# simonsysu/tfs

Hardware: AMD Instinct MI355X
Metric: GiB/s CRC32 verify, device-resident 64 KiB files; 1/2/4/8 MI355X (higher is better)
Workload: dtype u8

## Files before the change

### tfs_amd/csrc/tfs_ec_abi.cpp

```cpp
#include <hip/hip_runtime.h>

#include <cstdlib>
#include <cstring>
#include <mutex>
#include <vector>

#include "../../include/tfs_ec.h"
#include "crc_math.h"
#include "ec_math.h"

#include "ec_locate_plan.h"
#include "ec_marshal_plan.h"
#include "ec_read_plan.h"
#include "tfs_ec_device.h"

extern "C" int tfs_crc32_dev_malloc(tfs_crc_ctx* ctx, uint64_t bytes, void** d_ptr);
extern "C" int tfs_crc32_dev_free(tfs_crc_ctx* ctx, void* d_ptr);
extern "C" void* tfs_crc32_stream(tfs_crc_ctx* ctx);

using namespace tfsec;

namespace {
struct Plan {
  std::vector<int> sources, outputs;
// ... 147 lines not shown
    if (!dm[i]) dm[i] = ec->staging[p.sources[0]];
  rc = run_plan(ec, p, dm.data(), size, st);
  if (rc) return rc;
  for (int o : p.outputs)
    if (hipMemcpyAsync(members[o], dm[o], size_t(size), hipMemcpyDeviceToHost, st) != hipSuccess)
      return TFS_CRC_EXIT_DEVICE_ERROR;
  return hipStreamSynchronize(st) == hipSuccess ? TFS_SUCCESS : TFS_CRC_EXIT_DEVICE_ERROR;
}


const ReadTables& read_tables() {
  static const ReadTables* t = [] {
    ReadTables* r = new ReadTables();
    tfscrc::make_slice_tables(r->slice, 4);
    tfscrc::make_shift_table(r->step_packet, kReadStepPacket);
    tfscrc::make_shift_table(r->step_tile, kReadStepTile);
    const uint32_t g = tfscrc::x2nmodp(8, 0), gi = tfscrc::x2nmodp(0xFFFFFFFFull - 8, 0);
    r->xpow[kReadPowBias] = 1u << 31;
    for (int i = kReadPowBias + 1; i < kReadPowN; ++i) r->xpow[i] = tfscrc::multmodp(g, r->xpow[i - 1]);
    for (int i = kReadPowBias - 1; i >= 0; --i) r->xpow[i] = tfscrc::multmodp(gi, r->xpow[i + 1]);
    return r;
  }();
  return *t;
}

int upload_read_tables(tfs_ec* ec) {
  void* d = nullptr;
  const int rc = tfs_crc32_dev_malloc(ec->ctx, sizeof(ReadTables), &d);
  if (rc) return rc;
  if (hipMemcpy(d, &read_tables(), sizeof(ReadTables), hipMemcpyHostToDevice) != hipSuccess) {
    tfs_crc32_dev_free(ec->ctx, d);
    return TFS_CRC_EXIT_DEVICE_ERROR;
  }
  ec->d_read_tab = static_cast<ReadTables*>(d);
  return TFS_SUCCESS;
}

int check_read(tfs_ec* ec, void* const* members, const int* sizes, int size, int target, int* row) {
  const Plan& p = ec->dec;
  if (!p.valid || !ec->d_read_tab) return TFS_EXIT_MATRIX_INVALID;
  if (size < 0 || size % kUnit != 0) return TFS_EXIT_SIZE_INVALID;
  if (target < 0 || target >= ec->dn) return TFS_EXIT_PARAMETER_ERROR;
  *row = -1;
  for (size_t o = 0; o < p.outputs.size(); ++o)
    if (p.outputs[o] == target) *row = int(o);
  if (*row < 0) return TFS_EXIT_PARAMETER_ERROR;
  if (!members) return TFS_EXIT_DATA_INVALID;
  for (int s : p.sources)
    if (!members[s] || (sizes && sizes[s] < size)) return TFS_EXIT_DATA_INVALID;
  return TFS_SUCCESS;
}

int launch_read(tfs_ec* ec, void* const* members, int size, int row, const void* d_jobs, uint32_t n, void* d_out,
                uint64_t out_cap, uint32_t* d_out_crc, int32_t* d_out_status, uint32_t* d_n_bad, hipStream_t st) {
  const Plan& p = ec->dec;
  const int S = int(p.sources.size());
  ReadArgs a;
  memset(&a, 0, sizeof a);
  for (int s = 0; s < S; ++s) a.src[s] = static_cast<const uint8_t*>(members[p.sources[s]]);
  a.masks = p.d_masks + size_t(row) * 8 * size_t(S) * 8;
  a.tab = ec->d_read_tab;
  a.jobs = static_cast<const ReadJob*>(d_jobs);
  a.out = static_cast<uint8_t*>(d_out);
  a.out_cap = out_cap;
  a.out_crc = d_out_crc;
  a.out_status = d_out_status;
  a.n_bad = d_n_bad;
  a.n = n;
  a.S = uint32_t(S);
  a.size = size;
  return launch_ec_read(a, st) == hipSuccess ? TFS_SUCCESS : TFS_CRC_EXIT_DEVICE_ERROR;
}


const MarshalTables& marshal_tables() {
  static const MarshalTables* t = [] {
    MarshalTables* r = new MarshalTables();
    tfscrc::make_slice_tables(r->slice, 4);
    tfscrc::make_shift_table(r->step_packet, kReadStepPacket);
    const uint32_t g = tfscrc::x2nmodp(8, 0), gi = tfscrc::x2nmodp(0xFFFFFFFFull - 8, 0);
    r->xpow[kMarshalPowBias] = 1u << 31;
    for (int i = kMarshalPowBias + 1; i < kMarshalPowN; ++i) r->xpow[i] = tfscrc::multmodp(g, r->xpow[i - 1]);
    for (int i = kMarshalPowBias - 1; i >= 0; --i) r->xpow[i] = tfscrc::multmodp(gi, r->xpow[i + 1]);
    return r;
  }();
  return *t;
}

int chunk_check(tfs_ec_marshal* m, int offset, int len, hipStream_t want, hipStream_t* st) {
  if (!m || !m->ec) return TFS_EXIT_PARAMETER_ERROR;
  if (want == hipStreamPerThread) return TFS_EXIT_PARAMETER_ERROR;
  *st = want ? want : static_cast<hipStream_t>(tfs_crc32_stream(m->ec->ctx));
  if (m->stream_set && *st != m->stream) return TFS_EXIT_PARAMETER_ERROR;
  if (offset != m->next || len <= 0 || offset % 4096 != 0 || len % kUnit != 0 || len > m->total - offset)
    return TFS_EXIT_PARAMETER_ERROR;
  if (len % 4096 != 0 && offset + len != m->total) return TFS_EXIT_PARAMETER_ERROR;
  return TFS_SUCCESS;
}

int marshal_check(tfs_ec_marshal* m, void* const* members, int offset, int len, hipStream_t want, hipStream_t* st) {
  const int rc = chunk_check(m, offset, len, want, st);
  if (rc) return rc;
  if (!members) return TFS_EXIT_DATA_INVALID;
  for (int i = 0; i < m->ec->dn + m->ec->pn; ++i)
    if (!members[i]) return TFS_EXIT_DATA_INVALID;
  return TFS_SUCCESS;
}

int marshal_launch(tfs_ec_marshal* m, void* const* members, int offset, int len, hipStream_t st) {
  tfs_ec* ec = m->ec;
  const Plan& p = ec->enc;
  if (m->plan.recs.empty()) return run_plan(ec, p, members, len, st);
  const int S = int(p.sources.size());
  for (size_t o0 = 0; o0 < p.outputs.size(); o0 += kMaxOutGroup) {
    const int og = int(std::min<size_t>(kMaxOutGroup, p.outputs.size() - o0));
    MarshalArgs a;
    memset(&a, 0, sizeof a);
    for (int s = 0; s < S; ++s) a.ec.src[s] = static_cast<const uint8_t*>(members[p.sources[s]]);
    for (int o = 0; o < og; ++o) a.ec.dst[o] = static_cast<uint8_t*>(members[p.outputs[o0 + o]]);
    a.ec.masks = p.d_masks + o0 * 8 * size_t(S) * 8;
    a.ec.S = uint32_t(S);
    a.ec.units = uint64_t(len) / kUnit;
    if (o0) {
      if (launch_ec_apply(a.ec, og, 0, st) != hipSuccess) return TFS_CRC_EXIT_DEVICE_ERROR;
      continue;
    }
    a.tab = ec->d_marshal_tab;
    a.recs = m->d_recs;
    a.first = m->d_first;
    a.cont = m->d_cont;
    a.tail = m->d_tail;
    a.hdr = m->d_hdr;
    for (int s = 0; s < S; ++s) a.mend[s] = m->plan.mbegin[s + 1];
    a.tile0 = uint32_t(offset) >> 12;
    a.ntiles = m->plan.ntiles;
    if (launch_ec_marshal(a, og, st) != hipSuccess) return TFS_CRC_EXIT_DEVICE_ERROR;
  }
  return TFS_SUCCESS;
}


int reinstate_check(tfs_ec_reinstate* r, void* const* members, int offset, int len, hipStream_t want, hipStream_t* st) {
  if (!r) return TFS_EXIT_PARAMETER_ERROR;
  const int rc = chunk_check(&r->s, offset, len, want, st);
  if (rc) return rc;
  if (!members) return TFS_EXIT_DATA_INVALID;
  const Plan& p = r->s.ec->dec;
  for (int i : p.sources)
    if (!members[i]) return TFS_EXIT_DATA_INVALID;
  for (int i : p.outputs)
    if (!members[i]) return TFS_EXIT_DATA_INVALID;
  return TFS_SUCCESS;
}

int reinstate_launch(tfs_ec_reinstate* r, void* const* members, int offset, int len, hipStream_t st) {
  tfs_ec_marshal* m = &r->s;
  tfs_ec* ec = m->ec;
  const Plan& p = ec->dec;
  if (m->plan.recs.empty()) return run_plan(ec, p, members, len, st);
  const int S = int(p.sources.size()), dn = ec->dn;
  for (size_t o0 = 0; o0 < p.outputs.size(); o0 += kMaxOutGroup) {
    const int og = int(std::min<size_t>(kMaxOutGroup, p.outputs.size() - o0));
    ReinstateArgs a;
    memset(&a, 0, sizeof a);
    EcArgs& e = a.m.ec;
    for (int s = 0; s < S; ++s) e.src[s] = static_cast<const uint8_t*>(members[p.sources[s]]);
// ... 857 lines not shown
```

### tfs_amd/csrc/tfs_ec_device.h

```cpp
#pragma once
#include <hip/hip_runtime.h>
#include <stdint.h>

#include "ec_update_plan.h"

namespace tfsec {

constexpr int kMaxMembersDev = 12;
constexpr int kMaxOutGroup = 4;

struct EcArgs {
  const uint8_t* src[kMaxMembersDev];
  uint8_t* dst[kMaxOutGroup];
  const uint32_t* masks;
  uint32_t S;
  uint64_t units;
};

hipError_t launch_ec_apply(const EcArgs& a, int og, int variant, hipStream_t stream);

struct ReadJob {
  uint64_t file_id;
  uint64_t out_offset;
  int32_t offset, size;
  uint32_t flags, reserved;
};
static_assert(sizeof(ReadJob) == 32, "read job layout");
constexpr uint32_t kReadRange = 1u;
constexpr int kReadWaves = 8;
constexpr unsigned kReadMaxGrid = 4096;
constexpr uint32_t kReadStepPacket = 128, kReadStepTile = 4096u * kReadWaves - 896u;
constexpr int kReadPowBias = 4095;
constexpr int kReadPowN = kReadPowBias + 4096 * (kReadWaves - 1) + 3192 + 1;
struct ReadTables {
  uint32_t slice[4][256];
  uint32_t step_packet[4][256];
  uint32_t step_tile[4][256];
  uint32_t xpow[kReadPowN];
};
#ifdef __HIP__
__attribute__((host)) __attribute__((device))
#endif
inline int32_t read_job_check(const ReadJob& jb, int32_t member_size, uint64_t out_cap, uint32_t* A, uint32_t* E) {
  const int64_t cover_end = (int64_t(jb.offset) + int64_t(jb.size) + 1023) & ~int64_t(1023);
  if (jb.offset < 0 || jb.size < 0 || cover_end > int64_t(member_size)) return -1016;
  *A = uint32_t(jb.offset) & ~1023u;
  *E = uint32_t(cover_end);
  if ((jb.out_offset & 1023u) != 0u || jb.out_offset > out_cap || uint64_t(*E - *A) > out_cap - jb.out_offset)
    return -1016;
  if (!(jb.flags & kReadRange) && jb.size <= 36) return -8034;
  return 0;
}

struct ReadArgs {
  const uint8_t* src[kMaxMembersDev];
  const uint32_t* masks;
  const ReadTables* tab;
  const ReadJob* jobs;
  uint8_t* out;
  uint64_t out_cap;
  uint32_t* out_crc;
  int32_t* out_status;
  uint32_t* n_bad;
  uint32_t n, S;
  int32_t size;
};

hipError_t launch_ec_read(const ReadArgs& a, hipStream_t stream);

struct MarshalRec {
  uint32_t H, P1;
  uint32_t id_lo, id_hi;
};
constexpr int kMarshalPowBias = 4095;
constexpr int kMarshalPowN = kMarshalPowBias + 4096 + 1;
constexpr uint32_t kMarshalHdrWords = 9;
struct MarshalTables {
  uint32_t slice[4][256];
  uint32_t step_packet[4][256];
  uint32_t xpow[kMarshalPowN];
};
struct MarshalArgs {
  EcArgs ec;
  const MarshalTables* tab;
  const MarshalRec* recs;
  const uint32_t* first;
  uint32_t* cont;
  uint32_t* tail;
  uint32_t* hdr;
  uint32_t mend[kMaxMembersDev];
  uint32_t tile0;
  uint32_t ntiles;
};
hipError_t launch_ec_marshal(const MarshalArgs& a, int og, hipStream_t stream);

struct MarshalFoldArgs {
  const MarshalTables* tab;
  const MarshalRec* recs;
  const uint32_t* rec_member;
  const uint32_t* cont;
  const uint32_t* tail;
  const uint32_t* hdr;
  const uint32_t* pow_tile;
  uint32_t* out_crc;
  int32_t* out_status;
  uint32_t n, ntiles;
};
hipError_t launch_ec_marshal_fold(const MarshalFoldArgs& a, hipStream_t stream);

constexpr uint32_t kReinstateNoSlot = 0xFFFFFFFFu;
struct ReinstateArgs {
  MarshalArgs m;
  uint32_t src_slot[kMaxMembersDev];
  uint32_t out_slot[kMaxOutGroup];
};
hipError_t launch_ec_reinstate(const ReinstateArgs& a, int og, hipStream_t stream);

struct ScrubArgs {
  MarshalArgs m;
  const uint8_t* par[kMaxOutGroup];
  uint32_t* pbad;
  uint32_t o0;
};
hipError_t launch_ec_scrub(const ScrubArgs& a, int og, bool walk, hipStream_t stream);

struct ScrubCountArgs {
  const uint32_t* pbad;
  uint32_t* units;
  uint8_t* map;
  uint32_t ntiles;
};
hipError_t launch_ec_scrub_count(const ScrubCountArgs& a, int pn, hipStream_t stream);

struct LocateResult {
  int8_t kind, member;
  uint16_t parity, diff_bytes;
  uint8_t flags, zero;
};
static_assert(sizeof(LocateResult) == 8, "locate result layout");
constexpr int kLocateClean = 0, kLocateParity = 1, kLocateData = 2, kLocateNone = 3;
constexpr uint32_t kLocateConfirmed = 1u;
struct LocateArgs {
  const uint8_t* mem[kMaxMembersDev];
  const uint32_t* masks;
  const uint32_t* ratio;
  const uint32_t* inv0;
  const uint32_t* units;
  LocateResult* result;
  uint8_t* fixed;
  uint32_t n, dn, pn;
};
hipError_t launch_ec_locate(const LocateArgs& a, hipStream_t stream);

struct UpdateArgs {
  uint8_t* par[kMaxMembersDev];
  const uint32_t* masks;
  const uint32_t* units;
  const uint8_t* a;
  const uint8_t* b;
  uint32_t inl[kUpdateInline];
  uint32_t n, n_inline, dn, pn, member;
};
hipError_t launch_ec_update(const UpdateArgs& a, hipStream_t stream);

// ... 2 lines not shown
```

### tfs_amd/csrc/tfs_ec_kernels.hip

```cpp
#include <hip/hip_runtime.h>
#include <stdint.h>

#include "tfs_crc_device.h"
#include "tfs_ec_device.h"

namespace tfsec {

typedef unsigned int u32x2 __attribute__((ext_vector_type(2)));
typedef const __attribute__((address_space(1))) u32x2* gu64p;
typedef __attribute__((address_space(1))) u32x2* gu64wp;

__device__ __forceinline__ u32x2 ld64nt(const uint8_t* p) {
  return __builtin_nontemporal_load(reinterpret_cast<gu64p>(reinterpret_cast<uintptr_t>(p)));
}
__device__ __forceinline__ void st64nt(uint8_t* p, u32x2 v) {
  __builtin_nontemporal_store(v, reinterpret_cast<gu64wp>(reinterpret_cast<uintptr_t>(p)));
}
__device__ __forceinline__ uint32_t xand(uint32_t acc, uint32_t in, uint32_t m) {
  return __builtin_amdgcn_bitop3_b32(acc, in, m, 0x78);
}

template <int OG>
__device__ __forceinline__ void ec_apply_body(const EcArgs& a, const uint32_t* __restrict__ masks) {
  const int lane = threadIdx.x & 63;
// ... 314 lines not shown
            acc[r].x = xand(acc[r].x, in[c].x, mk);
            acc[r].y = xand(acc[r].y, in[c].y, mk);
          }
        }
#pragma unroll
        for (int c = 0; c < 8; ++c) in[c] = nx[c];
      }
      if (ok) {
#pragma unroll
        for (int r = 0; r < 8; ++r) st64nt(outp + (base - A) + 128u * r, acc[r]);
      }
      if (range) continue;
      if (t == 0) {
#pragma unroll
        for (int c = 0; c < 8; ++c) {
          const uint32_t q = base + 128u * c;
          if (q + 8u > H && q < P0) {
            const uint64_t v = uint64_t(acc[c].x) | (uint64_t(acc[c].y) << 32);
#pragma unroll
            for (int b = 0; b < 8; ++b) {
              const uint32_t p = q + uint32_t(b) - H;
              if (p < uint32_t(tfscrc::kFileInfoSize)) hdr8[p] = uint8_t(v >> (8 * b));
            }
          }
        }
      }
#pragma unroll
      for (int c = 0; c < 8; ++c) {
        const uint32_t q = base + 128u * c;
        uint32_t lo = acc[c].x, hi = acc[c].y;
        const int64_t sk = int64_t(P0) - int64_t(q), ek = int64_t(P1) - int64_t(q);
        if (sk > 0 || ek < 8) {
          const uint64_t mk = ek <= sk ? 0ull : rd_low_bytes(ek) & ~rd_low_bytes(sk);
          lo &= uint32_t(mk);
          hi &= uint32_t(mk >> 32);
        }
        const uint32_t piece = rd_slice4(sl, rd_slice4(sl, lo) ^ hi);
        crc = rd_lut4(c == 0 ? stt : stp, crc) ^ piece;
      }
    }
    if (range) {
      if (threadIdx.x == 0) {
        a.out_crc[j] = 0u;
        a.out_status[j] = tfscrc::kSuccess;
      }
      continue;
    }
    {
      const uint32_t tl = nt - 1u - ((nt - 1u - wv) & (kReadWaves - 1u));
      const int32_t dl = wv < nt ? int32_t(4096u * (nt - 1u - tl)) + 3192 - int32_t(1024u * u + off) : 0;
      const int32_t pad = int32_t(A + 4096u * nt - P1);
      crc = rd_multmodp(a.tab->xpow[kReadPowBias + dl - pad], crc);
#pragma unroll
      for (int m = 32; m >= 1; m >>= 1) crc ^= __shfl_xor(crc, m, 64);
      if (lane == 0) part[wv] = crc;
    }
    __syncthreads();
    if (threadIdx.x == 0) {
      uint32_t v = 0;
#pragma unroll
      for (int w = 0; w < kReadWaves; ++w) v ^= part[w];
      const uint64_t id = uint64_t(hdr[0]) | (uint64_t(hdr[1]) << 32);
      const int32_t fsize = int32_t(hdr[3]);
      const uint32_t fcrc = hdr[8];
      if (id != jb.file_id) status = tfscrc::kExitFileInfoError;
      else if (fsize != jb.size) status = tfscrc::kExitSyncFileError;
      else if (fcrc != v) status = tfscrc::kExitCheckCrcError;
      a.out_crc[j] = v;
      a.out_status[j] = status;
      if (status != tfscrc::kSuccess) ++bad;
    }
    __syncthreads();
  }
  if (threadIdx.x == 0 && bad && a.n_bad) atomicAdd(a.n_bad, bad);
}

hipError_t launch_ec_read(const ReadArgs& a, hipStream_t stream) {
  if (a.n == 0) return hipSuccess;
  const uint32_t blocks = a.n < kReadMaxGrid ? a.n : kReadMaxGrid;
  hipLaunchKernelGGL(ec_read_kernel, dim3(blocks), dim3(64 * kReadWaves), 0, stream, a);
  return hipGetLastError();
}

template <int OG>
__global__ void __launch_bounds__(256, OG <= 3 ? 4 : 3)
    ec_marshal_kernel(MarshalArgs a, const uint32_t* __restrict__ masks, const MarshalTables* __restrict__ tab,
                      const MarshalRec* __restrict__ recs, const uint32_t* __restrict__ first) {
  __shared__ uint32_t lt[2 * 1024];
  const uint32_t* sl = lt;
  const uint32_t* stp = lt + 1024;
  const int lane = threadIdx.x & 63;
  const uint32_t u = uint32_t(lane) >> 4;
  const uint32_t off = 8u * uint32_t(lane & 15);
  const uint32_t S = a.ec.S;
  const uint64_t ntl = (a.ec.units + 3) / 4;
  const uint64_t t = uint64_t(blockIdx.x) * 4u + __builtin_amdgcn_readfirstlane(threadIdx.x >> 6);
  const uint64_t unit = t * 4 + u;
  const bool ok = t < ntl && unit < a.ec.units;
  const uint64_t base = unit * 1024u + off;
  u32x2 in[8];
#pragma unroll
  for (int c = 0; c < 8; ++c) in[c] = ok ? ld64nt(a.ec.src[0] + base + 128u * c) : u32x2{0u, 0u};
  {
    const uint32_t* g = reinterpret_cast<const uint32_t*>(tab);
    for (uint32_t i = threadIdx.x; i < 2u * 1024u; i += 256u) lt[i] = g[i];
  }
  __syncthreads();
  if (t >= ntl) return;
  const uint32_t T = a.tile0 + uint32_t(t);
  const uint32_t tile_lo = T << 12, tile_hi = tile_lo + 4096u;
  const uint32_t q0 = tile_lo + 1024u * u + off;
  const int32_t dl = 3192 - int32_t(1024u * u + off);
  uint8_t* const hdr8 = reinterpret_cast<uint8_t*>(a.hdr);
  u32x2 acc[OG][8];
#pragma unroll
  for (int o = 0; o < OG; ++o)
#pragma unroll
    for (int r = 0; r < 8; ++r) acc[o][r] = u32x2{0u, 0u};
  for (uint32_t s = 0; s < S; ++s) {
    u32x2 nx[8];
    const bool more = s + 1 < S;
    const uint8_t* np = a.ec.src[more ? s + 1 : s];
#pragma unroll
    for (int c = 0; c < 8; ++c) nx[c] = (ok && more) ? ld64nt(np + base + 128u * c) : u32x2{0u, 0u};
#pragma unroll
    for (int o = 0; o < OG; ++o)
#pragma unroll
      for (int r = 0; r < 8; ++r) {
        const uint32_t* m = masks + ((uint32_t(o) * 8u + uint32_t(r)) * S + s) * 8u;
#pragma unroll
        for (int c = 0; c < 8; ++c) {
          const uint32_t mk = m[c];
          acc[o][r].x = xand(acc[o][r].x, in[c].x, mk);
          acc[o][r].y = xand(acc[o][r].y, in[c].y, mk);
        }
      }
    const uint32_t rend = a.mend[s];
    for (uint32_t r = __builtin_amdgcn_readfirstlane(first[size_t(s) * a.ntiles + T]); r < rend; ++r) {
      const uint32_t H = __builtin_amdgcn_readfirstlane(recs[r].H);
      const uint32_t P1 = __builtin_amdgcn_readfirstlane(recs[r].P1);
      if (H >= tile_hi) break;
      const uint32_t P0 = H + uint32_t(tfscrc::kFileInfoSize);
      const uint32_t live = 0u - uint32_t(P1 > tile_lo);
      if (P0 > tile_lo) {
#pragma unroll
        for (int c = 0; c < 8; ++c) {
          const uint32_t q = q0 + 128u * c;
          if (q + 8u > H && q < P0) {
            const uint64_t v = uint64_t(in[c].x & live) | (uint64_t(in[c].y & live) << 32);
#pragma unroll
            for (int b = 0; b < 8; ++b) {
              const uint32_t p = q + uint32_t(b) - H;
              if (p < uint32_t(tfscrc::kFileInfoSize)) hdr8[size_t(r) * (4u * kMarshalHdrWords) + p] = uint8_t(v >> (8 * b));
            }
          }
        }
      }
      if (P0 >= tile_hi) continue;
      uint32_t crc = 0;
      if (P0 <= tile_lo && P1 >= tile_hi) {
#pragma unroll
        for (int c = 0; c < 8; ++c) {
          const uint32_t piece = rd_slice4(sl, rd_slice4(sl, in[c].x & live) ^ (in[c].y & live));
          crc = c == 0 ? piece : rd_lut4(stp, crc) ^ piece;
        }
      } else {
#pragma unroll
        for (int c = 0; c < 8; ++c) {
          const uint32_t q = q0 + 128u * c;
          uint32_t lo = in[c].x & live, hi = in[c].y & live;
          const int64_t sk = int64_t(P0) - int64_t(q), ek = int64_t(P1) - int64_t(q);
          if (sk > 0 || ek < 8) {
            const uint64_t mk = ek <= sk ? 0ull : rd_low_bytes(ek) & ~rd_low_bytes(sk);
            lo &= uint32_t(mk);
            hi &= uint32_t(mk >> 32);
          }
          const uint32_t piece = rd_slice4(sl, rd_slice4(sl, lo) ^ hi);
          crc = c == 0 ? piece : rd_lut4(stp, crc) ^ piece;
        }
      }
      const bool on = P1 > tile_hi;
      const int32_t pad = P1 >= tile_hi ? 0 : int32_t(tile_hi - P1);
      crc = rd_multmodp(tab->xpow[kMarshalPowBias + dl - pad], crc);
#pragma unroll
      for (int m = 32; m >= 1; m >>= 1) crc ^= __shfl_xor(crc, m, 64);
      if (lane == 0) {
        if (on) a.cont[size_t(s) * a.ntiles + T] = crc;
        else a.tail[r] = crc;
      }
    }
#pragma unroll
    for (int c = 0; c < 8; ++c) in[c] = nx[c];
  }
  if (ok) {
#pragma unroll
    for (int o = 0; o < OG; ++o)
#pragma unroll
      for (int r = 0; r < 8; ++r) st64nt(a.ec.dst[o] + base + 128u * r, acc[o][r]);
  }
}

hipError_t launch_ec_marshal(const MarshalArgs& a, int og, hipStream_t stream) {
  if (a.ec.units == 0) return hipSuccess;
  const uint64_t ntl = (a.ec.units + 3) / 4;
  const dim3 g(static_cast<unsigned>((ntl + 3) / 4)), b(256);
  switch (og) {
    case 1: hipLaunchKernelGGL(ec_marshal_kernel<1>, g, b, 0, stream, a, a.ec.masks, a.tab, a.recs, a.first); break;
    case 2: hipLaunchKernelGGL(ec_marshal_kernel<2>, g, b, 0, stream, a, a.ec.masks, a.tab, a.recs, a.first); break;
    case 3: hipLaunchKernelGGL(ec_marshal_kernel<3>, g, b, 0, stream, a, a.ec.masks, a.tab, a.recs, a.first); break;
    default: hipLaunchKernelGGL(ec_marshal_kernel<4>, g, b, 0, stream, a, a.ec.masks, a.tab, a.recs, a.first); break;
  }
  return hipGetLastError();
}

__global__ void __launch_bounds__(256) ec_marshal_fold_kernel(MarshalFoldArgs a) {
  const uint32_t lane = threadIdx.x & 63u;
  const uint32_t r = blockIdx.x * 4u + __builtin_amdgcn_readfirstlane(threadIdx.x >> 6);
  if (r >= a.n) return;
  const MarshalRec rc = a.recs[r];
  const uint32_t P0 = rc.H + uint32_t(tfscrc::kFileInfoSize), P1 = rc.P1;
  const uint32_t t0 = P0 >> 12, tl = (P1 - 1u) >> 12;
  const uint32_t nc = tl - t0;
  uint32_t c = 0;
  if (nc) {
    const uint32_t* cont = a.cont + size_t(a.rec_member[r]) * a.ntiles;
    const uint32_t R = (nc + 63u) / 64u;
    const uint32_t b = min(t0 + lane * R, tl), e = min(b + R, tl);
    const uint32_t x4k = a.pow_tile[1];
    for (uint32_t t = b; t < e; ++t) c = rd_multmodp(x4k, c) ^ cont[t];
    c = rd_multmodp(a.pow_tile[tl - e], c);
#pragma unroll
    for (int m = 32; m >= 1; m >>= 1) c ^= __shfl_xor(c, m, 64);
  }
  if (lane == 0) {
    const uint32_t v = rd_multmodp(a.tab->xpow[kMarshalPowBias + int32_t(P1 - (tl << 12))], c) ^ a.tail[r];
    const uint32_t* h = a.hdr + size_t(r) * kMarshalHdrWords;
    const int32_t size = int32_t(P1 - rc.H);
    int32_t status = tfscrc::kSuccess;
    if (h[0] != rc.id_lo || h[1] != rc.id_hi) status = tfscrc::kExitFileInfoError;
    else if (int32_t(h[3]) != size) status = tfscrc::kExitSyncFileError;
    else if (h[8] != v) status = tfscrc::kExitCheckCrcError;
    a.out_crc[r] = v;
    a.out_status[r] = status;
  }
}

hipError_t launch_ec_marshal_fold(const MarshalFoldArgs& a, hipStream_t stream) {
  if (a.n == 0) return hipSuccess;
  hipLaunchKernelGGL(ec_marshal_fold_kernel, dim3((a.n + 3u) / 4u), dim3(256), 0, stream, a);
  return hipGetLastError();
}

struct ReinstateWalk {
  const uint32_t* sl;
  const uint32_t* stp;
  uint32_t T, tile_lo, tile_hi, q0, ntiles;
  int32_t dl;
  int lane;
};

template <bool QREC = false>
__device__ __forceinline__ void reinstate_walk(const u32x2 (&pc)[8], const ReinstateWalk& w, uint32_t slot, uint32_t rend,
                                               const MarshalTables* __restrict__ tab, const MarshalRec* __restrict__ recs,
                                               const uint32_t* __restrict__ first, uint32_t* cont, uint32_t* tail,
                                               uint8_t* hdr8) {
  const uint32_t tile_lo = w.tile_lo, tile_hi = w.tile_hi;
  for (uint32_t r = __builtin_amdgcn_readfirstlane(first[size_t(slot) * w.ntiles + w.T]); r < rend; ++r) {
    const uint32_t H = __builtin_amdgcn_readfirstlane(recs[r].H);
    const uint32_t P1 = __builtin_amdgcn_readfirstlane(recs[r].P1);
    if (H >= tile_hi) break;
    const uint32_t P0 = H + uint32_t(tfscrc::kFileInfoSize);
    const uint32_t live = 0u - uint32_t(P1 > tile_lo);
    const uint32_t q0 = QREC ? w.q0 + ~live : w.q0;
    if (P0 > tile_lo) {
#pragma unroll
      for (int c = 0; c < 8; ++c) {
        const uint32_t q = q0 + 128u * c;
        if (q + 8u > H && q < P0) {
          const uint64_t v = uint64_t(pc[c].x & live) | (uint64_t(pc[c].y & live) << 32);
#pragma unroll
          for (int b = 0; b < 8; ++b) {
            const uint32_t p = q + uint32_t(b) - H;
            if (p < uint32_t(tfscrc::kFileInfoSize)) hdr8[size_t(r) * (4u * kMarshalHdrWords) + p] = uint8_t(v >> (8 * b));
          }
        }
      }
    }
    if (P0 >= tile_hi) continue;
    uint32_t crc = 0;
    if (P0 <= tile_lo && P1 >= tile_hi) {
#pragma unroll
      for (int c = 0; c < 8; ++c) {
        const uint32_t piece = rd_slice4(w.sl, rd_slice4(w.sl, pc[c].x & live) ^ (pc[c].y & live));
        crc = c == 0 ? piece : rd_lut4(w.stp, crc) ^ piece;
      }
    } else {
#pragma unroll
      for (int c = 0; c < 8; ++c) {
        const uint32_t q = q0 + 128u * c;
        uint32_t lo = pc[c].x & live, hi = pc[c].y & live;
        const int64_t sk = int64_t(P0) - int64_t(q), ek = int64_t(P1) - int64_t(q);
        if (sk > 0 || ek < 8) {
          const uint64_t mk = ek <= sk ? 0ull : rd_low_bytes(ek) & ~rd_low_bytes(sk);
          lo &= uint32_t(mk);
          hi &= uint32_t(mk >> 32);
        }
        const uint32_t piece = rd_slice4(w.sl, rd_slice4(w.sl, lo) ^ hi);
        crc = c == 0 ? piece : rd_lut4(w.stp, crc) ^ piece;
      }
    }
    const bool on = P1 > tile_hi;
    const int32_t pad = P1 >= tile_hi ? 0 : int32_t(tile_hi - P1);
    crc = rd_multmodp(tab->xpow[kMarshalPowBias + w.dl - pad], crc);
#pragma unroll
    for (int m = 32; m >= 1; m >>= 1) crc ^= __shfl_xor(crc, m, 64);
    if (w.lane == 0) {
      if (on) cont[size_t(slot) * w.ntiles + w.T] = crc;
      else tail[r] = crc;
    }
  }
}

template <int OG>
__global__ void __launch_bounds__(256, OG <= 2 ? 4 : 3)
    ec_reinstate_kernel(ReinstateArgs a, const uint32_t* __restrict__ masks, const MarshalTables* __restrict__ tab,
                        const MarshalRec* __restrict__ recs, const uint32_t* __restrict__ first) {
  __shared__ uint32_t lt[2 * 1024];
  const int lane = threadIdx.x & 63;
  const uint32_t u = uint32_t(lane) >> 4;
  const uint32_t off = 8u * uint32_t(lane & 15);
  const uint32_t S = a.m.ec.S;
  const uint64_t ntl = (a.m.ec.units + 3) / 4;
  const uint64_t t = uint64_t(blockIdx.x) * 4u + __builtin_amdgcn_readfirstlane(threadIdx.x >> 6);
  const uint64_t unit = t * 4 + u;
  const bool ok = t < ntl && unit < a.m.ec.units;
  const uint64_t base = unit * 1024u + off;
  u32x2 in[8];
#pragma unroll
  for (int c = 0; c < 8; ++c) in[c] = ok ? ld64nt(a.m.ec.src[0] + base + 128u * c) : u32x2{0u, 0u};
  {
    const uint32_t* g = reinterpret_cast<const uint32_t*>(tab);
    for (uint32_t i = threadIdx.x; i < 2u * 1024u; i += 256u) lt[i] = g[i];
  }
  __syncthreads();
  if (t >= ntl) return;
  ReinstateWalk w;
  w.sl = lt;
  w.stp = lt + 1024;
  w.T = a.m.tile0 + uint32_t(t);
  w.tile_lo = w.T << 12;
  w.tile_hi = w.tile_lo + 4096u;
  w.q0 = w.tile_lo + 1024u * u + off;
  w.ntiles = a.m.ntiles;
  w.dl = 3192 - int32_t(1024u * u + off);
  w.lane = lane;
  uint8_t* const hdr8 = reinterpret_cast<uint8_t*>(a.m.hdr);
  u32x2 acc[OG][8];
#pragma unroll
  for (int o = 0; o < OG; ++o)
#pragma unroll
    for (int r = 0; r < 8; ++r) acc[o][r] = u32x2{0u, 0u};
  for (uint32_t s = 0; s < S; ++s) {
    u32x2 nx[8];
    const bool more = s + 1 < S;
    const uint8_t* np = a.m.ec.src[more ? s + 1 : s];
#pragma unroll
    for (int c = 0; c < 8; ++c) nx[c] = (ok && more) ? ld64nt(np + base + 128u * c) : u32x2{0u, 0u};
#pragma unroll
    for (int o = 0; o < OG; ++o)
#pragma unroll
      for (int r = 0; r < 8; ++r) {
        const uint32_t* m = masks + ((uint32_t(o) * 8u + uint32_t(r)) * S + s) * 8u;
#pragma unroll
        for (int c = 0; c < 8; ++c) {
          const uint32_t mk = m[c];
          acc[o][r].x = xand(acc[o][r].x, in[c].x, mk);
          acc[o][r].y = xand(acc[o][r].y, in[c].y, mk);
        }
      }
    const uint32_t slot = a.src_slot[s];
    if (slot != kReinstateNoSlot) reinstate_walk(in, w, slot, a.m.mend[slot], tab, recs, first, a.m.cont, a.m.tail, hdr8);
#pragma unroll
    for (int c = 0; c < 8; ++c) in[c] = nx[c];
  }
  if (ok) {
#pragma unroll
    for (int o = 0; o < OG; ++o)
#pragma unroll
      for (int r = 0; r < 8; ++r) st64nt(a.m.ec.dst[o] + base + 128u * r, acc[o][r]);
  }
#pragma unroll
  for (int o = 0; o < OG; ++o) {
    const uint32_t slot = a.out_slot[o];
    if (slot != kReinstateNoSlot) reinstate_walk(acc[o], w, slot, a.m.mend[slot], tab, recs, first, a.m.cont, a.m.tail, hdr8);
  }
}

hipError_t launch_ec_reinstate(const ReinstateArgs& a, int og, hipStream_t stream) {
  if (a.m.ec.units == 0) return hipSuccess;
  const uint64_t ntl = (a.m.ec.units + 3) / 4;
  const dim3 g(static_cast<unsigned>((ntl + 3) / 4)), b(256);
  switch (og) {
    case 1: hipLaunchKernelGGL(ec_reinstate_kernel<1>, g, b, 0, stream, a, a.m.ec.masks, a.m.tab, a.m.recs, a.m.first); break;
    case 2: hipLaunchKernelGGL(ec_reinstate_kernel<2>, g, b, 0, stream, a, a.m.ec.masks, a.m.tab, a.m.recs, a.m.first); break;
    case 3: hipLaunchKernelGGL(ec_reinstate_kernel<3>, g, b, 0, stream, a, a.m.ec.masks, a.m.tab, a.m.recs, a.m.first); break;
    default: hipLaunchKernelGGL(ec_reinstate_kernel<4>, g, b, 0, stream, a, a.m.ec.masks, a.m.tab, a.m.recs, a.m.first); break;
  }
  return hipGetLastError();
}

__device__ __forceinline__ u32x2 ld64nt_at(const uint8_t* p, uint32_t o) {
  typedef const __attribute__((address_space(1))) uint8_t* g8p;
  return __builtin_nontemporal_load(reinterpret_cast<gu64p>(reinterpret_cast<g8p>(reinterpret_cast<uintptr_t>(p)) + o));
}

template <int OG, bool WALK>
__global__ void __launch_bounds__(256, OG <= 3 ? 4 : 3)
    ec_scrub_kernel(ScrubArgs a, const uint32_t* __restrict__ masks, const MarshalTables* __restrict__ tab,
                    const MarshalRec* __restrict__ recs, const uint32_t* __restrict__ first) {
  __shared__ uint32_t lt[WALK ? 2 * 1024 : 1];
  const int lane = threadIdx.x & 63;
  const uint32_t u = uint32_t(lane) >> 4;
  const uint32_t off = 8u * uint32_t(lane & 15);
  const uint32_t S = a.m.ec.S;
  __builtin_assume(S != 0u);
  const uint64_t ntl = (a.m.ec.units + 3) / 4;
  const uint64_t t = uint64_t(blockIdx.x) * 4u + __builtin_amdgcn_readfirstlane(threadIdx.x >> 6);
  const uint64_t unit = t * 4 + u;
  const bool ok = t < ntl && unit < a.m.ec.units;
  const uint32_t base = uint32_t(unit) * 1024u + off;
  u32x2 in[8];
#pragma unroll
  for (int c = 0; c < 8; ++c) in[c] = ok ? ld64nt_at(a.m.ec.src[0], base + 128u * c) : u32x2{0u, 0u};
  if (WALK) {
    const uint32_t* g = reinterpret_cast<const uint32_t*>(tab);
    for (uint32_t i = threadIdx.x; i < 2u * 1024u; i += 256u) lt[i] = g[i];
    __syncthreads();
  }
  if (t >= ntl) return;
  const uint32_t T = a.m.tile0 + uint32_t(t);
  ReinstateWalk w;
  w.sl = lt;
  w.stp = lt + (WALK ? 1024 : 0);
  w.T = T;
  w.tile_lo = T << 12;
  w.tile_hi = w.tile_lo + 4096u;
  w.q0 = w.tile_lo + 1024u * u + off;
  w.ntiles = a.m.ntiles;
  w.dl = 3192 - int32_t(1024u * u + off);
  w.lane = lane;
  uint8_t* const hdr8 = reinterpret_cast<uint8_t*>(a.m.hdr);
  u32x2 acc[OG][8];
#pragma unroll
  for (int o = 0; o < OG; ++o)
#pragma unroll
    for (int r = 0; r < 8; ++r) acc[o][r] = u32x2{0u, 0u};
  for (uint32_t s = 0; s < S; ++s) {
    u32x2 nx[8];
    const uint8_t* np = s + 1 < S ? a.m.ec.src[s + 1] : a.par[0];
#pragma unroll
    for (int c = 0; c < 8; ++c) nx[c] = ok ? ld64nt_at(np, base + 128u * c) : u32x2{0u, 0u};
#pragma unroll
    for (int o = 0; o < OG; ++o)
#pragma unroll
      for (int r = 0; r < 8; ++r) {
        const uint32_t* m = masks + ((uint32_t(o) * 8u + uint32_t(r)) * S + s) * 8u;
#pragma unroll
        for (int c = 0; c < 8; ++c) {
          const uint32_t mk = m[c];
          acc[o][r].x = xand(acc[o][r].x, in[c].x, mk);
          acc[o][r].y = xand(acc[o][r].y, in[c].y, mk);
        }
      }
    if (WALK) reinstate_walk<true>(in, w, s, a.m.mend[s], tab, recs, first, a.m.cont, a.m.tail, hdr8);
#pragma unroll
    for (int c = 0; c < 8; ++c) in[c] = nx[c];
  }
#pragma unroll
  for (int o = 0; o < OG; ++o) {
    u32x2 nx[8];
#pragma unroll
    for (int c = 0; c < 8; ++c) nx[c] = (ok && o + 1 < OG) ? ld64nt_at(a.par[o + 1 < OG ? o + 1 : o], base + 128u * c) : u32x2{0u, 0u};
    uint32_t d = 0;
#pragma unroll
    for (int r = 0; r < 8; ++r) d |= (acc[o][r].x ^ in[r].x) | (acc[o][r].y ^ in[r].y);
    const uint64_t b = __builtin_amdgcn_ballot_w64(d != 0u);
    const uint32_t bits = uint32_t((b & 0xFFFFull) != 0ull) | (uint32_t(((b >> 16) & 0xFFFFull) != 0ull) << 1) |
                          (uint32_t(((b >> 32) & 0xFFFFull) != 0ull) << 2) | (uint32_t((b >> 48) != 0ull) << 3);
    if (__builtin_amdgcn_mbcnt_hi(~0u, __builtin_amdgcn_mbcnt_lo(~0u, 0u)) == 0u) a.pbad[size_t(a.o0 + uint32_t(o)) * a.m.ntiles + T] = bits;
#pragma unroll
    for (int c = 0; c < 8; ++c) in[c] = nx[c];
  }
}

template <bool WALK>
static void launch_scrub_og(const ScrubArgs& a, int og, dim3 g, dim3 b, hipStream_t stream) {
  switch (og) {
    case 1: hipLaunchKernelGGL((ec_scrub_kernel<1, WALK>), g, b, 0, stream, a, a.m.ec.masks, a.m.tab, a.m.recs, a.m.first); break;
    case 2: hipLaunchKernelGGL((ec_scrub_kernel<2, WALK>), g, b, 0, stream, a, a.m.ec.masks, a.m.tab, a.m.recs, a.m.first); break;
    case 3: hipLaunchKernelGGL((ec_scrub_kernel<3, WALK>), g, b, 0, stream, a, a.m.ec.masks, a.m.tab, a.m.recs, a.m.first); break;
    default: hipLaunchKernelGGL((ec_scrub_kernel<4, WALK>), g, b, 0, stream, a, a.m.ec.masks, a.m.tab, a.m.recs, a.m.first); break;
  }
}

hipError_t launch_ec_scrub(const ScrubArgs& a, int og, bool walk, hipStream_t stream) {
  if (a.m.ec.units == 0) return hipSuccess;
  const uint64_t ntl = (a.m.ec.units + 3) / 4;
  const dim3 g(static_cast<unsigned>((ntl + 3) / 4)), b(256);
  if (walk) launch_scrub_og<true>(a, og, g, b, stream);
  else launch_scrub_og<false>(a, og, g, b, stream);
  return hipGetLastError();
}

__global__ void __launch_bounds__(1024) ec_scrub_count_kernel(ScrubCountArgs a) {
  __shared__ uint32_t part[16];
  const uint32_t p = blockIdx.x;
  const uint32_t* w = a.pbad + size_t(p) * a.ntiles;
  uint8_t* mp = a.map + size_t(p) * a.ntiles;
  uint32_t c = 0;
  for (uint32_t T0 = threadIdx.x; T0 < a.ntiles; T0 += 4096u) {
    uint32_t v[4];
#pragma unroll
    for (int k = 0; k < 4; ++k) v[k] = T0 + 1024u * k < a.ntiles ? w[T0 + 1024u * k] & 15u : 0u;
#pragma unroll
    for (int k = 0; k < 4; ++k)
      if (T0 + 1024u * k < a.ntiles) {
        mp[T0 + 1024u * k] = uint8_t(v[k]);
        c += uint32_t(__popc(v[k]));
      }
  }
#pragma unroll
  for (int m = 32; m >= 1; m >>= 1) c += __shfl_xor(c, m, 64);
// ... 251 lines not shown
```

Measured before the change: 6296.

## Replace per-lane CRC shift and shuffle reduction with staged LDS lane-shift tables and DPP

The per-record CRC combine across a wave's 64 lanes used to do a per-lane multiply by a power of x from a global table, followed by a six-step shfl_xor butterfly. It now runs a three-level hierarchical combine: 5-bit-indexed shift tables staged in LDS, DPP xors within quads and rows, and four readlanes. The final pad adjustment is applied once to the combined value, and only when the record ends inside the tile. This targets the global-table multiply and the cross-lane shuffle latency in the marshal, reinstate and scrub record walks. In exchange, LDS use per block grows by about 10 KiB, which may lower occupancy, and the staging load per block gets larger.

```diff
diff --git a/tfs_amd/csrc/tfs_ec_abi.cpp b/tfs_amd/csrc/tfs_ec_abi.cpp
--- a/tfs_amd/csrc/tfs_ec_abi.cpp
+++ b/tfs_amd/csrc/tfs_ec_abi.cpp
@@ -253,6 +253,8 @@
     r->xpow[kMarshalPowBias] = 1u << 31;
     for (int i = kMarshalPowBias + 1; i < kMarshalPowN; ++i) r->xpow[i] = tfscrc::multmodp(g, r->xpow[i - 1]);
     for (int i = kMarshalPowBias - 1; i >= 0; --i) r->xpow[i] = tfscrc::multmodp(gi, r->xpow[i + 1]);
+    for (int lv = 0; lv < 3; ++lv)
+      for (int k = 0; k < 4; ++k) tfscrc::make_shift_table5(r->lane_shift[lv][k],uint64_t(kMarshalLaneStep[lv]) * uint64_t(3 - k));
     return r;
   }();
   return *t;
diff --git a/tfs_amd/csrc/tfs_ec_device.h b/tfs_amd/csrc/tfs_ec_device.h
--- a/tfs_amd/csrc/tfs_ec_device.h
+++ b/tfs_amd/csrc/tfs_ec_device.h
@@ -1,5 +1,6 @@
 #pragma once
 #include <hip/hip_runtime.h>
+#include <stddef.h>
 #include <stdint.h>
 
 #include "ec_update_plan.h"
@@ -75,11 +76,17 @@
 constexpr int kMarshalPowBias = 4095;
 constexpr int kMarshalPowN = kMarshalPowBias + 4096 + 1;
 constexpr uint32_t kMarshalHdrWords = 9;
+constexpr uint32_t kMarshalLaneStep[3] = {8, 32, 1024};
+constexpr uint32_t kMarshalLaneWords = 3 * 4 * 7 * 32;
+constexpr uint32_t kMarshalStageWords = 2 * 1024 + kMarshalLaneWords;
 struct MarshalTables {
   uint32_t slice[4][256];
   uint32_t step_packet[4][256];
   uint32_t xpow[kMarshalPowN];
+  uint32_t lane_shift[3][4][7][32];
 };
+static_assert(sizeof(MarshalTables::lane_shift) == 4 * kMarshalLaneWords && kMarshalLaneWords % 4 == 0, "lane_shift layout");
+static_assert(offsetof(MarshalTables, lane_shift) % 16 == 0, "lane_shift is staged in 16-byte pieces");
 struct MarshalArgs {
   EcArgs ec;
   const MarshalTables* tab;
diff --git a/tfs_amd/csrc/tfs_ec_kernels.hip b/tfs_amd/csrc/tfs_ec_kernels.hip
--- a/tfs_amd/csrc/tfs_ec_kernels.hip
+++ b/tfs_amd/csrc/tfs_ec_kernels.hip
@@ -420,13 +420,51 @@
   return hipGetLastError();
 }
 
+template <int CTRL>
+__device__ __forceinline__ uint32_t dpp_xor(uint32_t v) {
+  return v ^ uint32_t(__builtin_amdgcn_update_dpp(0, int(v), CTRL, 0xF, 0xF, false));
+}
+__device__ __forceinline__ uint32_t rd_lut5(const uint32_t* t, uint32_t x) {
+  uint32_t v[7];
+#pragma unroll
+  for (int k = 0; k < 7; ++k) v[k] = t[32u * k + ((x >> (5 * k)) & 31u)];
+  __builtin_amdgcn_sched_group_barrier(0x100, 7, 0);
+  return v[0] ^ v[1] ^ v[2] ^ v[3] ^ v[4] ^ v[5] ^ v[6];
+}
+__device__ __forceinline__ uint32_t marshal_combine(const uint32_t* ls, uint32_t crc) {
+  constexpr uint32_t kT = 7u * 32u;
+  const uint32_t l = __builtin_amdgcn_mbcnt_hi(~0u, __builtin_amdgcn_mbcnt_lo(~0u, 0u));
+  crc = rd_lut5(ls + (l & 3u) * kT, crc);
+  crc = dpp_xor<0xB1>(crc);
+  crc = dpp_xor<0x4E>(crc);
+  crc = rd_lut5(ls + (4u + ((l >> 2) & 3u)) * kT, crc);
+  crc = dpp_xor<0x124>(crc);
+  crc = dpp_xor<0x128>(crc);
+  crc = rd_lut5(ls + (8u + (l >> 4)) * kT, crc);
+  return uint32_t(__builtin_amdgcn_readlane(int(crc), 0)) ^ uint32_t(__builtin_amdgcn_readlane(int(crc), 16)) ^
+         uint32_t(__builtin_amdgcn_readlane(int(crc), 32)) ^ uint32_t(__builtin_amdgcn_readlane(int(crc), 48));
+}
+__device__ __forceinline__ void marshal_stage(uint32_t* lt, const MarshalTables* __restrict__ tab) {
+  const uint4* g = reinterpret_cast<const uint4*>(tab);
+  const uint4* gl = reinterpret_cast<const uint4*>(&tab->lane_shift[0][0][0][0]);
+  uint4* d = reinterpret_cast<uint4*>(lt);
+  constexpr uint32_t kN = kMarshalLaneWords / 4u;
+#pragma unroll
+  for (uint32_t i = 0; i < 2u * 256u; i += 256u) d[i + threadIdx.x] = g[i + threadIdx.x];
+#pragma unroll
+  for (uint32_t i = 0; i < kN; i += 256u) {
+    const uint32_t j = min(i + threadIdx.x, kN - 1u);
+    d[2u * 256u + j] = gl[j];
+  }
+}
 template <int OG>
 __global__ void __launch_bounds__(256, OG <= 3 ? 4 : 3)
     ec_marshal_kernel(MarshalArgs a, const uint32_t* __restrict__ masks, const MarshalTables* __restrict__ tab,
                       const MarshalRec* __restrict__ recs, const uint32_t* __restrict__ first) {
-  __shared__ uint32_t lt[2 * 1024];
+  __shared__ alignas(16) uint32_t lt[kMarshalStageWords];
   const uint32_t* sl = lt;
   const uint32_t* stp = lt + 1024;
+  const uint32_t* lsh = lt + 2048;
   const int lane = threadIdx.x & 63;
   const uint32_t u = uint32_t(lane) >> 4;
   const uint32_t off = 8u * uint32_t(lane & 15);
@@ -439,16 +477,12 @@
   u32x2 in[8];
 #pragma unroll
   for (int c = 0; c < 8; ++c) in[c] = ok ? ld64nt(a.ec.src[0] + base + 128u * c) : u32x2{0u, 0u};
-  {
-    const uint32_t* g = reinterpret_cast<const uint32_t*>(tab);
-    for (uint32_t i = threadIdx.x; i < 2u * 1024u; i += 256u) lt[i] = g[i];
-  }
+  marshal_stage(lt, tab);
   __syncthreads();
   if (t >= ntl) return;
   const uint32_t T = a.tile0 + uint32_t(t);
   const uint32_t tile_lo = T << 12, tile_hi = tile_lo + 4096u;
   const uint32_t q0 = tile_lo + 1024u * u + off;
-  const int32_t dl = 3192 - int32_t(1024u * u + off);
   uint8_t* const hdr8 = reinterpret_cast<uint8_t*>(a.hdr);
   u32x2 acc[OG][8];
 #pragma unroll
@@ -474,9 +508,10 @@
         }
       }
     const uint32_t rend = a.mend[s];
-    for (uint32_t r = __builtin_amdgcn_readfirstlane(first[size_t(s) * a.ntiles + T]); r < rend; ++r) {
-      const uint32_t H = __builtin_amdgcn_readfirstlane(recs[r].H);
-      const uint32_t P1 = __builtin_amdgcn_readfirstlane(recs[r].P1);
+    for (uint32_t rv = first[size_t(s) * a.ntiles + T]; rv < rend; ++rv) {
+      const uint32_t r = __builtin_amdgcn_readfirstlane(rv);
+      const uint32_t H = recs[r].H;
+      const uint32_t P1 = recs[r].P1;
       if (H >= tile_hi) break;
       const uint32_t P0 = H + uint32_t(tfscrc::kFileInfoSize);
       const uint32_t live = 0u - uint32_t(P1 > tile_lo);
@@ -518,13 +553,11 @@
         }
       }
       const bool on = P1 > tile_hi;
-      const int32_t pad = P1 >= tile_hi ? 0 : int32_t(tile_hi - P1);
-      crc = rd_multmodp(tab->xpow[kMarshalPowBias + dl - pad], crc);
-#pragma unroll
-      for (int m = 32; m >= 1; m >>= 1) crc ^= __shfl_xor(crc, m, 64);
+      uint32_t seg = marshal_combine(lsh, crc);
+      if (P1 < tile_hi) seg = rd_multmodp(tab->xpow[kMarshalPowBias - int32_t(tile_hi - P1)], seg);
       if (lane == 0) {
-        if (on) a.cont[size_t(s) * a.ntiles + T] = crc;
-        else a.tail[r] = crc;
+        if (on) a.cont[size_t(s) * a.ntiles + T] = seg;
+        else a.tail[r] = seg;
       }
     }
 #pragma unroll
@@ -592,8 +625,8 @@
 struct ReinstateWalk {
   const uint32_t* sl;
   const uint32_t* stp;
+  const uint32_t* lsh;
   uint32_t T, tile_lo, tile_hi, q0, ntiles;
-  int32_t dl;
   int lane;
 };
 
@@ -603,9 +636,10 @@
                                                const uint32_t* __restrict__ first, uint32_t* cont, uint32_t* tail,
                                                uint8_t* hdr8) {
   const uint32_t tile_lo = w.tile_lo, tile_hi = w.tile_hi;
-  for (uint32_t r = __builtin_amdgcn_readfirstlane(first[size_t(slot) * w.ntiles + w.T]); r < rend; ++r) {
-    const uint32_t H = __builtin_amdgcn_readfirstlane(recs[r].H);
-    const uint32_t P1 = __builtin_amdgcn_readfirstlane(recs[r].P1);
+  for (uint32_t rv = first[size_t(slot) * w.ntiles + w.T]; rv < rend; ++rv) {
+    const uint32_t r = __builtin_amdgcn_readfirstlane(rv);
+    const uint32_t H = recs[r].H;
+    const uint32_t P1 = recs[r].P1;
     if (H >= tile_hi) break;
     const uint32_t P0 = H + uint32_t(tfscrc::kFileInfoSize);
     const uint32_t live = 0u - uint32_t(P1 > tile_lo);
@@ -648,13 +682,11 @@
       }
     }
     const bool on = P1 > tile_hi;
-    const int32_t pad = P1 >= tile_hi ? 0 : int32_t(tile_hi - P1);
-    crc = rd_multmodp(tab->xpow[kMarshalPowBias + w.dl - pad], crc);
-#pragma unroll
-    for (int m = 32; m >= 1; m >>= 1) crc ^= __shfl_xor(crc, m, 64);
+    uint32_t seg = marshal_combine(w.lsh, crc);
+    if (P1 < tile_hi) seg = rd_multmodp(tab->xpow[kMarshalPowBias - int32_t(tile_hi - P1)], seg);
     if (w.lane == 0) {
-      if (on) cont[size_t(slot) * w.ntiles + w.T] = crc;
-      else tail[r] = crc;
+      if (on) cont[size_t(slot) * w.ntiles + w.T] = seg;
+      else tail[r] = seg;
     }
   }
 }
@@ -663,7 +695,7 @@
 __global__ void __launch_bounds__(256, OG <= 2 ? 4 : 3)
     ec_reinstate_kernel(ReinstateArgs a, const uint32_t* __restrict__ masks, const MarshalTables* __restrict__ tab,
                         const MarshalRec* __restrict__ recs, const uint32_t* __restrict__ first) {
-  __shared__ uint32_t lt[2 * 1024];
+  __shared__ alignas(16) uint32_t lt[kMarshalStageWords];
   const int lane = threadIdx.x & 63;
   const uint32_t u = uint32_t(lane) >> 4;
   const uint32_t off = 8u * uint32_t(lane & 15);
@@ -676,21 +708,18 @@
   u32x2 in[8];
 #pragma unroll
   for (int c = 0; c < 8; ++c) in[c] = ok ? ld64nt(a.m.ec.src[0] + base + 128u * c) : u32x2{0u, 0u};
-  {
-    const uint32_t* g = reinterpret_cast<const uint32_t*>(tab);
-    for (uint32_t i = threadIdx.x; i < 2u * 1024u; i += 256u) lt[i] = g[i];
-  }
+  marshal_stage(lt, tab);
   __syncthreads();
   if (t >= ntl) return;
   ReinstateWalk w;
   w.sl = lt;
   w.stp = lt + 1024;
+  w.lsh = lt + 2048;
   w.T = a.m.tile0 + uint32_t(t);
   w.tile_lo = w.T << 12;
   w.tile_hi = w.tile_lo + 4096u;
   w.q0 = w.tile_lo + 1024u * u + off;
   w.ntiles = a.m.ntiles;
-  w.dl = 3192 - int32_t(1024u * u + off);
   w.lane = lane;
   uint8_t* const hdr8 = reinterpret_cast<uint8_t*>(a.m.hdr);
   u32x2 acc[OG][8];
@@ -756,7 +785,7 @@
 __global__ void __launch_bounds__(256, OG <= 3 ? 4 : 3)
     ec_scrub_kernel(ScrubArgs a, const uint32_t* __restrict__ masks, const MarshalTables* __restrict__ tab,
                     const MarshalRec* __restrict__ recs, const uint32_t* __restrict__ first) {
-  __shared__ uint32_t lt[WALK ? 2 * 1024 : 1];
+  __shared__ alignas(16) uint32_t lt[WALK ? kMarshalStageWords : 4];
   const int lane = threadIdx.x & 63;
   const uint32_t u = uint32_t(lane) >> 4;
   const uint32_t off = 8u * uint32_t(lane & 15);
@@ -771,8 +800,7 @@
 #pragma unroll
   for (int c = 0; c < 8; ++c) in[c] = ok ? ld64nt_at(a.m.ec.src[0], base + 128u * c) : u32x2{0u, 0u};
   if (WALK) {
-    const uint32_t* g = reinterpret_cast<const uint32_t*>(tab);
-    for (uint32_t i = threadIdx.x; i < 2u * 1024u; i += 256u) lt[i] = g[i];
+    marshal_stage(lt, tab);
     __syncthreads();
   }
   if (t >= ntl) return;
@@ -780,12 +808,12 @@
   ReinstateWalk w;
   w.sl = lt;
   w.stp = lt + (WALK ? 1024 : 0);
+  w.lsh = lt + (WALK ? 2048 : 0);
   w.T = T;
   w.tile_lo = T << 12;
   w.tile_hi = w.tile_lo + 4096u;
   w.q0 = w.tile_lo + 1024u * u + off;
   w.ntiles = a.m.ntiles;
-  w.dl = 3192 - int32_t(1024u * u + off);
   w.lane = lane;
   uint8_t* const hdr8 = reinterpret_cast<uint8_t*>(a.m.hdr);
   u32x2 acc[OG][8];
```

New measurement: 6204. 0.985x the previous value.
